# usebeforefree/reed-solomon-cc

Hardware: AMD Instinct MI355X
Metric: device-resident encode+reconstruct GiB/s per GPU (RS(10,4), 1 MiB shards); % HBM roofline (higher is better)
Workload: dtype u8

## Files before the change

include/reedsol.h:

```cpp
#ifndef REEDSOL_AMD_H
#define REEDSOL_AMD_H

#include <stddef.h>
#include <stdint.h>

#ifdef __cplusplus
extern "C" {
#endif

typedef enum rs_status {
  RS_OK = 0,
  RS_ERR_TOO_FEW_ORIGINAL_SHARDS = 1,
  RS_ERR_NOT_ENOUGH_SHARDS = 2,
  RS_ERR_INVALID_SHARD_SIZE = 3,
  RS_ERR_UNSUPPORTED_SHARD_COUNT = 4,
  RS_ERR_TOO_MANY_ORIGINAL_SHARDS = 5,
  RS_ERR_DIFFERENT_SHARD_SIZE = 6,
  RS_ERR_INVALID_SHARD_INDEX = 7,
  RS_ERR_DUPLICATE_SHARD_INDEX = 8,
  RS_ERR_TOO_MANY_SHARDS = 9,
  RS_ERR_OUT_OF_MEMORY = 10,
  RS_ERR_OVERFLOW = 11,
  RS_ERR_LOW_RATE_UNSUPPORTED = 12,
  RS_ERR_SHARD_TAIL_UNSUPPORTED = 13,
// ... 74 lines not shown
                        uint32_t max_u, const uint32_t *d_index, uint64_t index_stride, const void *d_old,
                        const void *d_new, uint64_t change_stripe_stride, void *d_recovery,
                        uint64_t recovery_stripe_stride, int32_t *d_status, uint32_t flags, rs_stream_t stream);
int rs_update_selftest(uint64_t original_count, uint64_t recovery_count, uint32_t max_u, int trials, uint64_t seed,
                       uint64_t *mismatches);

int rs_rebuild_batch_dev(uint64_t original_count, uint64_t recovery_count, size_t shard_bytes, uint64_t n_stripes,
                         const uint8_t *d_present, uint64_t present_stride, uint32_t max_e,
                         const void *d_original, uint64_t original_stripe_stride,
                         const void *d_recovery, uint64_t recovery_stripe_stride,
                         void *d_rebuilt, uint64_t rebuilt_stripe_stride, int32_t *d_status,
                         uint32_t flags, rs_stream_t stream);
const char *rs_rebuild_kernel_name(uint64_t k, uint64_t m, size_t shard_bytes, uint32_t max_e);
int rs_rebuild_compile_check(uint64_t k, uint64_t m, double *compile_ms, uint64_t *code_bytes);
int rs_rebuild_selftest(uint64_t k, uint64_t m, int trials, uint64_t seed, uint64_t *mismatches);

int rs_encode_batch_host(uint64_t original_count, uint64_t recovery_count, size_t shard_bytes, uint64_t n_stripes,
                         const void *h_original, uint64_t original_stripe_stride, void *h_recovery,
                         uint64_t recovery_stripe_stride, uint32_t flags);
int rs_reconstruct_batch_host(uint64_t original_count, uint64_t recovery_count, size_t shard_bytes,
                              uint64_t n_stripes, const uint8_t *present, const void *h_original,
                              uint64_t original_stripe_stride, const void *h_recovery,
                              uint64_t recovery_stripe_stride, void *h_restored, uint64_t restored_stripe_stride,
                              uint32_t flags);

int rs_encode_batch_host_multi(uint64_t original_count, uint64_t recovery_count, size_t shard_bytes,
                               uint64_t n_stripes, const void *h_original, uint64_t original_stripe_stride,
                               void *h_recovery, uint64_t recovery_stripe_stride, uint32_t flags,
                               const int *devices, int n_devices);
int rs_reconstruct_batch_host_multi(uint64_t original_count, uint64_t recovery_count, size_t shard_bytes,
                                    uint64_t n_stripes, const uint8_t *present, const void *h_original,
                                    uint64_t original_stripe_stride, const void *h_recovery,
                                    uint64_t recovery_stripe_stride, void *h_restored,
                                    uint64_t restored_stripe_stride, uint32_t flags, const int *devices,
                                    int n_devices);

const char *rs_encode_kernel_name(uint64_t original_count, uint64_t recovery_count, size_t shard_bytes);
const char *rs_reconstruct_kernel_name(uint64_t original_count, uint64_t recovery_count, size_t shard_bytes,
                                       const uint8_t *present);
const char *rs_patterns_kernel_name(uint64_t original_count, uint64_t recovery_count, size_t shard_bytes,
                                    uint32_t max_e, uint32_t flags);

int rs_net_wait(void);

int rs_reconstruct_warm(uint64_t original_count, uint64_t recovery_count, size_t shard_bytes, const uint8_t *present,
                        uint32_t flags);

const char *rs_last_kernels(void);

int64_t rs_debug_fail_alloc(int64_t n);
int rs_debug_release_caches(uint64_t *pooled_contexts);
int64_t rs_debug_erasure_logs_check(uint64_t k, uint64_t m, const uint8_t *received, int low);
int rs_debug_fft_stamps(uint64_t *out, uint64_t n);

int rs_jit_stats(uint64_t *compiles, uint64_t *cache_hits, uint64_t *modules);

int rs_net_compile_check(uint64_t original_count, uint64_t recovery_count, const uint8_t *present,
                         uint32_t flags, double *compile_ms);

int rs_psyn_compile_check(uint64_t original_count, uint64_t recovery_count, uint32_t flags, double *compile_ms,
                          uint64_t *code_bytes);
int rs_fft_compile_check(uint64_t original_count, uint64_t recovery_count, uint32_t flags, double *compile_ms,
                         uint64_t *code_bytes, uint64_t *valu_ops);
int rs_fft_selftest(uint64_t original_count, uint64_t recovery_count, uint32_t flags, const uint8_t *skip,
                    int trials, uint64_t *mismatches);

int rs_fft_decode_compile_check(uint64_t original_count, uint64_t recovery_count, double *compile_ms,
                                uint64_t *code_bytes);
int rs_fft_pdecode_compile_check(uint64_t original_count, uint64_t recovery_count, const uint8_t *present,
                                 double *compile_ms, uint64_t *code_bytes);
int rs_fft_decode_selftest(uint64_t original_count, uint64_t recovery_count, uint32_t erased, int trials,
                           uint64_t *mismatches);

int rs_lowrate_selftest(uint64_t original_count, uint64_t recovery_count, int trials, uint64_t seed,
                        uint64_t *mismatches);

int rs_engine_fft(uint8_t *shards, uint64_t shard_count, size_t shard_bytes, uint64_t pos, uint64_t size,
                  uint64_t truncated_size, uint64_t skew_delta, uint32_t flags);
int rs_engine_ifft(uint8_t *shards, uint64_t shard_count, size_t shard_bytes, uint64_t pos, uint64_t size,
                   uint64_t truncated_size, uint64_t skew_delta, uint32_t flags);
int rs_engine_mul_scalar(uint8_t *chunks, size_t bytes, uint16_t log_m, uint32_t flags);
int rs_engine_eval_poly(uint16_t *erasures, uint64_t truncated_size);

const uint16_t *rs_table_exp(void);
const uint16_t *rs_table_log(void);
const uint16_t *rs_table_skew(void);
const uint16_t *rs_table_log_walsh(void);
const uint8_t *rs_table_mul_128(void);


#ifdef __cplusplus
}
#endif
#endif
```

reed-solomon-cc_amd/csrc/rs_fftnet.cpp:

```cpp
#include "rs_fftnet.hpp"

#include <algorithm>
#include <cstdio>
#include <cstring>
#include <map>
#include <mutex>
#include <random>
#include <sstream>

#include "reedsol.h"
#include "rs_env.hpp"
#include "rs_gf.hpp"
#include "rs_internal.hpp"

namespace rs {
namespace fftnet {
namespace {

struct Basis {
  bool ok = false;
  uint8_t p[8] = {};
};

const Basis &basis() {
  static const Basis b = [] {
    Basis r;
    const Tables &t = tables();
    r.ok = true;
    for (int i = 0; i < 8; i++) {
      const uint16_t prod = mul16(static_cast<uint16_t>(1u << 8), t.log[1u << i]);
      const uint16_t pi = static_cast<uint16_t>((1u << (8 + i)) ^ prod);
      if (pi >> 8) r.ok = false;
      r.p[i] = static_cast<uint8_t>(pi);
    }
    return r;
  }();
  return b;
}

uint16_t to_uv(uint16_t x) {
  const Basis &b = basis();
  uint8_t lo = 0;
  for (int i = 0; i < 8; i++)
    if (x >> (8 + i) & 1) lo ^= b.p[i];
  return static_cast<uint16_t>(x ^ lo);
}

struct Tw {
  bool zero = true;
  bool sub = false;
  uint8_t A[8] = {}, B[8] = {}, Cm[8] = {}, D[8] = {};
};

Tw twiddle(uint16_t log_m, bool d1) {
  Tw t;
  if (log_m == kModulus) return t;
  t.zero = false;
  for (int j = 0; j < 8; j++) {
    const uint16_t cu = to_uv(mul_engine(to_uv(static_cast<uint16_t>(1u << j)), log_m, d1));
    const uint16_t cv = to_uv(mul_engine(to_uv(static_cast<uint16_t>(1u << (8 + j))), log_m, d1));
    for (int i = 0; i < 8; i++) {
      t.A[i] |= static_cast<uint8_t>((cu >> i & 1) << j);
      t.Cm[i] |= static_cast<uint8_t>((cu >> (8 + i) & 1) << j);
      t.B[i] |= static_cast<uint8_t>((cv >> i & 1) << j);
      t.D[i] |= static_cast<uint8_t>((cv >> (8 + i) & 1) << j);
    }
  }
  t.sub = true;
  for (int i = 0; i < 8; i++)
    if (t.B[i] || t.Cm[i] || t.A[i] != t.D[i]) t.sub = false;
  return t;
}

struct Bf {
  uint32_t x, y;
  uint16_t log_m;
};
struct Layer {
  int bit;
  bool inv;
  std::vector<Bf> bf;
};

uint16_t sk(uint64_t idx) { return idx < kModulus ? tables().skew[idx] : static_cast<uint16_t>(kModulus); }

uint16_t gmul_elem(uint16_t x, uint16_t y) { return x && y ? mul16(x, tables().log[y]) : 0; }

int log2i(uint64_t v) {
  int b = 0;
  while ((1ull << b) < v) b++;
  return b;
}

std::vector<Layer> ifft_layers(uint64_t size, uint64_t trunc, uint64_t sd) {
  std::vector<Layer> out;
  uint64_t d = 1;
  for (uint64_t d4 = 4; d4 <= size; d = d4, d4 <<= 2) {
    Layer l1{log2i(d), true, {}}, l2{log2i(d) + 1, true, {}};
    for (uint64_t r = 0; r < trunc; r += d4) {
      const uint64_t b = r + d + sd - 1;
      const uint16_t m01 = sk(b), m02 = sk(b + d), m23 = sk(b + 2 * d);
      for (uint64_t i = r; i < r + d; i++) {
        l1.bf.push_back({uint32_t(i), uint32_t(i + d), m01});
        l1.bf.push_back({uint32_t(i + 2 * d), uint32_t(i + 3 * d), m23});
        l2.bf.push_back({uint32_t(i), uint32_t(i + 2 * d), m02});
        l2.bf.push_back({uint32_t(i + d), uint32_t(i + 3 * d), m02});
      }
    }
    out.push_back(std::move(l1));
    out.push_back(std::move(l2));
  }
  if (d < size) {
    Layer l{log2i(d), true, {}};
    const uint16_t lm = sk(d + sd - 1);
    for (uint64_t i = 0; i < d; i++) l.bf.push_back({uint32_t(i), uint32_t(d + i), lm});
    out.push_back(std::move(l));
  }
  return out;
}

std::vector<Layer> fft_layers(uint64_t size, uint64_t trunc, uint64_t sd) {
  std::vector<Layer> out;
  uint64_t d4 = size;
  for (uint64_t d = size >> 2; d != 0; d4 = d, d >>= 2) {
// ... 172 lines not shown
#endif
  u32 s[8], o[8];
#pragma unroll
  for (int j = 0; j < 8; j++) s[j] = SWN(x[j]);
#pragma unroll
  for (int i0 = 0; i0 < 8; i0 += RS_RMUL_G) {
    u32 m[16 * RS_RMUL_G];
#pragma unroll
    for (int t = 0; t < 16 * RS_RMUL_G; t++) m[t] = M[16 * i0 + t];
#pragma unroll
    for (int g = 0; g < RS_RMUL_G; g++) {
      u32 a = x[0] & m[16 * g];
#pragma unroll
      for (int j = 1; j < 8; j++) a = __builtin_amdgcn_bitop3_b32(a, x[j], m[16 * g + j], 0x78);
#pragma unroll
      for (int j = 0; j < 8; j++) a = __builtin_amdgcn_bitop3_b32(a, s[j], m[16 * g + 8 + j], 0x78);
      o[i0 + g] = a;
    }
  }
#pragma unroll
  for (int i = 0; i < 8; i++) x[i] = o[i];
}
)HIP";

int sched_of() { return 1; }

int prefetch_of(const Spec &s) {
  return std::max(0, std::min(8, s.prefetch >= 0 ? s.prefetch : env::num(env::FFT_PREFETCH)));
}

int debug_of() { return env::num(env::FFT_DEBUG); }

std::mutex g_stamp_mu;
std::map<int, unsigned long long *> g_stamp_bufs;
unsigned long long *stamp_buffer(int dev) {
  std::lock_guard<std::mutex> lk(g_stamp_mu);
  unsigned long long *&p = g_stamp_bufs[dev];
  if (!p && hipMalloc(reinterpret_cast<void **>(&p), 8 * 64 * 8) == hipSuccess) (void)hipMemset(p, 0, 8 * 64 * 8);
  return p;
}


struct Gen {
  std::ostringstream o;
  int tmp = 0;
  Stats *st = nullptr;
  uint64_t *ops = nullptr;

  std::string fresh(const char *p = "zt") { return p + std::to_string(tmp++); }
  void op(uint64_t n = 1) {
    if (ops) *ops += n;
  }

  void rows(const std::vector<std::string> &ins, const std::vector<uint32_t> &rowmask,
            const std::vector<std::string> &dst, bool acc) {
    std::vector<std::string> names = ins;
    std::vector<std::vector<int>> r(rowmask.size());
    for (size_t i = 0; i < rowmask.size(); i++)
      for (size_t j = 0; j < ins.size(); j++)
        if (rowmask[i] >> j & 1) r[i].push_back(static_cast<int>(j));
    for (;;) {
      std::map<std::pair<int, int>, int> cnt;
      for (auto &row : r)
        for (size_t a = 0; a < row.size(); a++)
          for (size_t b = a + 1; b < row.size(); b++) cnt[{std::min(row[a], row[b]), std::max(row[a], row[b])}]++;
      std::pair<int, int> best{-1, -1};
      int bc = 1;
      for (auto &kv : cnt)
        if (kv.second > bc) {
          bc = kv.second;
          best = kv.first;
        }
      if (best.first < 0) break;
      const std::string nm = fresh();
      o << "  const u32 " << nm << " = " << names[best.first] << " ^ " << names[best.second] << ";\n";
      op();
      const int id = static_cast<int>(names.size());
      names.push_back(nm);
      for (auto &row : r) {
        auto ia = std::find(row.begin(), row.end(), best.first), ib = std::find(row.begin(), row.end(), best.second);
        if (ia != row.end() && ib != row.end()) {
          row.erase(std::remove_if(row.begin(), row.end(), [&](int v) { return v == best.first || v == best.second; }),
                    row.end());
          row.push_back(id);
        }
      }
    }
    for (size_t i = 0; i < r.size(); i++) {
      std::vector<std::string> t;
      for (int id : r[i]) t.push_back(names[id]);
      const std::string &d = dst[i];
      size_t at = 0;
      if (!acc) {
        if (t.empty()) {
          o << "  " << d << " = 0u;\n";
          continue;
        }
        if (t.size() == 1) {
          o << "  " << d << " = " << t[0] << ";\n";
          continue;
        }
        if (t.size() == 2 || t.size() == 4) {
          o << "  " << d << " = " << t[0] << " ^ " << t[1] << ";\n";
          at = 2;
        } else {
          o << "  " << d << " = X3(" << t[0] << ", " << t[1] << ", " << t[2] << ");\n";
          at = 3;
        }
        op();
      }
      for (; at + 1 < t.size(); at += 2) {
        o << "  " << d << " = X3(" << d << ", " << t[at] << ", " << t[at + 1] << ");\n";
        op();
      }
      if (at < t.size()) {
        o << "  " << d << " ^= " << t[at] << ";\n";
        op();
      }
    }
  }

  static std::vector<std::string> regs(const std::string &pfx) {
    std::vector<std::string> v;
    for (int i = 0; i < 8; i++) v.push_back(pfx + "_" + std::to_string(i));
    return v;
  }

  void mul(const std::vector<std::string> &dst, bool acc, const std::vector<std::string> &src, const Tw &t) {
    if (t.sub) {
      if (st) st->subfield++;
      std::vector<uint32_t> rm(8);
      for (int i = 0; i < 8; i++) rm[i] = t.A[i];
      rows(src, rm, dst, acc);
      return;
    }
    if (st) st->general++;
    std::vector<std::string> ins = src;
    for (int j = 0; j < 8; j++) {
      const std::string s = fresh("zs");
      o << "  const u32 " << s << " = SWN(" << src[j] << ");\n";
      op(3);
      ins.push_back(s);
    }
    std::vector<uint32_t> rm(16);
    std::vector<std::string> tl(16);
    for (int i = 0; i < 8; i++) {
      rm[i] = t.A[i] | (uint32_t(t.B[i]) << 8);
      rm[8 + i] = t.D[i] | (uint32_t(t.Cm[i]) << 8);
      tl[i] = fresh("zl");
      tl[8 + i] = fresh("zh");
    }
    o << "  u32 ";
    for (int i = 0; i < 16; i++) o << tl[i] << (i < 15 ? ", " : ";\n");
    rows(ins, rm, tl, false);
    for (int i = 0; i < 8; i++) {
      if (acc)
        o << "  " << dst[i] << " ^= MUX(" << tl[i] << ", " << tl[8 + i] << ", KM.f);\n";
      else
        o << "  " << dst[i] << " = MUX(" << tl[i] << ", " << tl[8 + i] << ", KM.f);\n";
      op(acc ? 2 : 1);
    }
  }

  void pin(const std::vector<std::string> &v) {
    o << "  asm volatile(\"\" :";
    for (size_t i = 0; i < v.size(); i++) o << (i ? ", " : " ") << "\"+v\"(" << v[i] << ")";
    o << ");\n";
  }

  void copy(const std::vector<std::string> &dst, const std::vector<std::string> &src) {
    for (int i = 0; i < 8; i++) o << "  " << dst[i] << " = " << src[i] << ";\n";
  }
  void xor_into(const std::vector<std::string> &dst, const std::vector<std::string> &src) {
    for (int i = 0; i < 8; i++) o << "  " << dst[i] << " ^= " << src[i] << ";\n";
    op(8);
  }

  int sched = 0;
  int nbf = 0;

  void butterfly(const std::string &xn, bool &zx, const std::string &yn, bool &zy, bool inv, const Tw &t) {
    const auto X = regs(xn), Y = regs(yn);
    if (zx && zy) return;
    if (sched && ++nbf % sched == 0) o << "  __builtin_amdgcn_sched_barrier(0);\n";
    if (t.zero && st) st->xor_only++;
    if (inv) {
      if (!zx) {
        if (zy)
          copy(Y, X);
        else
          xor_into(Y, X);
        zy = false;
      }
      if (!t.zero && !zy) {
        mul(X, !zx, Y, t);
        zx = false;
      }
    } else {
      if (!t.zero && !zy) {
        mul(X, !zx, Y, t);
        zx = false;
      }
      if (!zx) {
        if (zy)
          copy(Y, X);
        else
          xor_into(Y, X);
        zy = false;
      }
    }
  }

  void basis_change(const std::vector<std::string> &d) {
    const Basis &b = basis();
    std::vector<std::string> h(8), nn(8);
    for (int i = 0; i < 8; i++) {
      h[i] = fresh("zv");
      o << "  const u32 " << h[i] << " = " << d[i] << " >> 4;\n";
      op();
    }
    std::vector<uint32_t> rm(8, 0);
    for (int j = 0; j < 8; j++)
      for (int i = 0; i < 8; i++)
        if (b.p[i] >> j & 1) rm[j] |= 1u << i;
    o << "  u32 ";
    for (int j = 0; j < 8; j++) {
      nn[j] = fresh("zn");
      o << nn[j] << (j < 7 ? ", " : ";\n");
    }
    rows(h, rm, nn, false);
    for (int j = 0; j < 8; j++)
      if (rm[j]) {
        o << "  " << d[j] << " = XM(" << d[j] << ", " << nn[j] << ");\n";
        op();
      }
  }
};

std::string wname(uint32_t r) { return "w" + std::to_string(r); }
std::string bname(uint32_t t) { return "b" + std::to_string(t); }
std::string cname(uint32_t t) { return "c" + std::to_string(t); }

std::string mask_expr(const std::vector<uint32_t> &per_wave) {
  bool same = true;
  for (uint32_t v : per_wave) same &= v == per_wave[0];
  if (same) return std::to_string(per_wave[0]) + "u";
  std::string e = "0u";
  for (size_t w = per_wave.size(); w-- > 0;)
    e = "(w == " + std::to_string(w) + "u ? " + std::to_string(per_wave[w]) + "u : " + e + ")";
  return e;
}

uint32_t dyn_store_word(const Plan &P) { return static_cast<uint32_t>((P.truncs.size() * P.C + 31) / 32); }

std::string gen_source(const Spec &s, const std::string &name, Stats *stats) {
  Plan P = make_plan(s);
  Gen g;
  g.st = stats;
  g.sched = sched_of();
  Stats dummy;
  if (!g.st) g.st = &dummy;
  std::ostringstream &o = g.o;
  const uint32_t NW = P.NW, C = P.C;
  bool any_xor = s.decode;
  for (uint32_t q = 0; q < s.m; q++) any_xor |= P.out_mode[q] == kOutXorRec;
  const bool dyn = s.dyn;
  const int dbg = debug_of();
  const bool old_order = s.decode && (dbg & 16);
  const bool tail = s.decode && !(dbg & 4);
  const bool spat = s.decode && !s.present.empty();
  std::vector<uint8_t> inR(C, 0);
  std::vector<uint16_t> lp_log(C, 0);
  std::vector<int32_t> out_row(s.k, -1);
  std::vector<uint32_t> cg_log(s.k, 0);
  if (spat) {
    const Tables &T = tables();
    uint32_t e = 0, nr = 0;
// ... 1054 lines not shown
  };
  auto rmul = [](uint16_t x, const uint32_t *M) -> uint16_t {
    const uint8_t u = x & 0xFF, v = x >> 8;
    uint16_t r = 0;
    for (int i = 0; i < 8; i++) {
      int lo = 0, hi = 0;
      for (int j = 0; j < 8; j++) {
        lo ^= ((u >> j & 1) && (M[16 * i + j] & 0x0F0F0F0Fu)) ^ ((v >> j & 1) && (M[16 * i + 8 + j] & 0x0F0F0F0Fu));
        hi ^= ((v >> j & 1) && (M[16 * i + j] & 0xF0F0F0F0u)) ^ ((u >> j & 1) && (M[16 * i + 8 + j] & 0xF0F0F0F0u));
      }
      r |= static_cast<uint16_t>(lo << i | hi << (8 + i));
    }
    return r;
  };
  std::vector<uint32_t> blk(decode_block_words(s));
  for (int tr = 0; tr < trials; tr++) {
    std::vector<uint16_t> data(k), par(m);
    for (auto &x : data) x = static_cast<uint16_t>(rng());
    scalar_encode(data.data(), k, m, false, false, par.data());
    std::vector<uint8_t> present(k + m, 1);
    std::vector<uint32_t> idx(k);
    for (uint32_t i = 0; i < k; i++) idx[i] = i;
    std::shuffle(idx.begin(), idx.end(), rng);
    for (uint32_t i = 0; i < e; i++) present[idx[i]] = 0;
    for (uint32_t p = 0; p < m - e; p++)
      if (rng() % 4 == 0) present[k + rng() % m] = 0;
    uint32_t have = 0;
    for (uint32_t p = 0; p < m; p++) have += present[k + p];
    if (have < e) continue;
    if (decode_block(s, present.data(), blk.data()) != RS_OK) return ~0ull;
    std::vector<uint16_t> d2 = data, enc(m);
    for (uint32_t g = 0; g < k; g++)
      if (!present[g]) d2[g] = 0;
    scalar_encode(d2.data(), k, m, false, false, enc.data());
    std::vector<uint16_t> a(C, 0);
    for (uint32_t p = 0; p < m; p++)
      if (blk[dwm + 1 + p / 32] >> (p % 32) & 1) a[p] = rmul(to_uv(par[p] ^ enc[p]), &blk[mko + 128 * p]);
    for (const Layer &L : ifft_layers(C, m, 0)) apply(a, L);
    for (uint32_t K = 1; K <= (k + C - 1) / C; K++) {
      if (!(blk[dwm] >> K & 1)) continue;
      const uint32_t tK = std::min<uint32_t>(C, k - (K - 1) * C);
      std::vector<uint16_t> y = a;
      for (const Layer &L : fft_layers(C, tK, static_cast<uint64_t>(K) * C)) apply(y, L);
      for (uint32_t q = 0; q < tK; q++) {
        const uint32_t g = (K - 1) * C + q;
        if (present[g]) continue;
        bad += to_uv(rmul(y[q], &blk[mko + 128 * (m + g)])) != data[g];
      }
    }
  }
  return bad;
}

}
}
```

reed-solomon-cc_amd/csrc/rs_fftnet.hpp:

```cpp
#pragma once
#include <hip/hip_runtime.h>

#include <cstdint>
#include <string>
#include <vector>

#include "rs_jit.hpp"

namespace rs {
namespace fftnet {

constexpr uint8_t kOutNone = 0;
constexpr uint8_t kOutStore = 1;
constexpr uint8_t kOutXorRec = 2;

struct Spec {
  uint32_t k = 0, m = 0;
  uint32_t flags = 0;
  std::vector<uint8_t> skip;
  std::vector<uint8_t> out_mode;
  int prefetch = -1;
  uint32_t pieces = 1;
  bool inverse = false;
  bool dyn = false;
  bool decode = false;
  bool blocked = false;
  std::vector<uint8_t> present;
};
uint32_t dyn_mask_words(const Spec &s);

bool supports_inverse(uint64_t k, uint64_t m, uint64_t shard_bytes);

constexpr uint64_t kUnitBytes = 2048;

constexpr uint32_t kMaxChunks = 16;
bool supports(uint64_t k, uint64_t m, uint64_t shard_bytes, bool chunk16 = false);
uint32_t pieces(uint64_t shard_bytes);

std::string generate(const Spec &s, const std::string &name);
std::string cache_key(const Spec &s);
std::string kernel_name(const Spec &s);

const jit::Kernel *get(const Spec &s, bool async, std::string &err, bool &pending);
bool compile_check(const Spec &s, std::string &err, double *ms, size_t *code_bytes);

hipError_t launch(const jit::Kernel &kn, const Spec &s, const uint8_t *data, uint64_t ds, const uint8_t *rec, uint64_t rs,
                  uint8_t *out, uint64_t os, uint64_t sb, uint64_t n_stripes, hipStream_t st,
                  const uint32_t *dmask = nullptr, uint32_t dmask_words = 0, bool shared_mask = false);

uint32_t decode_block_words(const Spec &s);
uint32_t decode_mask_offset(const Spec &s);
bool decode_betas(uint32_t k, uint32_t m, std::vector<uint16_t> &beta);
void scalar_masks(uint16_t c, uint32_t *masks);
void uv_basis(uint32_t p[8]);
int decode_block(const Spec &s, const uint8_t *present, uint32_t *blk);
uint64_t decode_selftest(uint32_t k, uint32_t m, uint32_t e, int trials);

uint64_t selftest(const Spec &s, int trials);
int read_stamps(uint64_t *host, size_t n);

struct Stats {
  uint64_t ops_a = 0, ops_b = 0, ops_io = 0, subfield = 0, general = 0, xor_only = 0;
};
Stats stats(const Spec &s);

}
}
```

reed-solomon-cc_amd/csrc/rs_plans.cpp:

```cpp
#include "rs_host.hpp"

namespace rs {
namespace host {

PlanCache<EncodePlan> g_enc_plans;
PlanCache<DecodePlan> g_dec_plans;

void release_plans() {
  std::lock_guard<std::mutex> lk(g_plan_mu);
  g_enc_plans.clear();
  g_dec_plans.clear();
}

void encode_map(uint64_t k, uint64_t m, uint32_t flags, jit::NetSpec &ns) {
  const bool d1 = flags & RS_FLAG_QUIRK_D1, d2 = flags & RS_FLAG_QUIRK_D2;
  ns.role = "encode";
  ns.n_in = static_cast<uint32_t>(k);
  ns.n_out = static_cast<uint32_t>(m);
  ns.src.clear();
  ns.images.assign(k * m * 16, 0);
  std::vector<uint16_t> in(k, 0), out(m);
  for (uint64_t t = 0; t < k; t++) {
    ns.src.push_back(static_cast<int32_t>(t));
    for (int b = 0; b < 16; b++) {
// ... 487 lines not shown
    return RS_OK;
  });
}

int rs_fft_decode_compile_check(uint64_t k, uint64_t m, double *compile_ms, uint64_t *code_bytes) {
  return guarded([&]() -> int {
    int st = check_codec(k, m, fftnet::kUnitBytes);
    if (st) return st;
    if (!fftnet::supports(k, m, fftnet::kUnitBytes, true)) return fail(RS_ERR_INVALID_ARGUMENT, "no FFT kernel form");
    fftnet::Spec spec;
    spec.k = static_cast<uint32_t>(k);
    spec.m = static_cast<uint32_t>(m);
    spec.dyn = spec.decode = true;
    std::string err;
    size_t bytes = 0;
    if (!fftnet::compile_check(spec, err, compile_ms, &bytes)) return fail(RS_ERR_DEVICE, err);
    if (code_bytes) *code_bytes = bytes;
    return RS_OK;
  });
}

int rs_fft_pdecode_compile_check(uint64_t k, uint64_t m, const uint8_t *present, double *compile_ms,
                                 uint64_t *code_bytes) {
  return guarded([&]() -> int {
    int st = check_codec(k, m, fftnet::kUnitBytes);
    if (st) return st;
    if (!present) return fail(RS_ERR_INVALID_ARGUMENT, "present == NULL");
    if (!fftnet::supports(k, m, fftnet::kUnitBytes, true)) return fail(RS_ERR_INVALID_ARGUMENT, "no FFT kernel form");
    uint64_t e = 0, have = 0;
    for (uint64_t i = 0; i < k; i++) e += present[i] ? 0 : 1;
    for (uint64_t i = 0; i < m; i++) have += present[k + i] ? 1 : 0;
    if (have < e) return fail(RS_ERR_NOT_ENOUGH_SHARDS, "fewer than original_count shards present");
    if (e == 0) return fail(RS_ERR_INVALID_ARGUMENT, "nothing erased");
    fftnet::Spec spec;
    spec.k = static_cast<uint32_t>(k);
    spec.m = static_cast<uint32_t>(m);
    spec.decode = true;
    spec.present.assign(present, present + k + m);
    std::string err;
    size_t bytes = 0;
    if (!fftnet::compile_check(spec, err, compile_ms, &bytes)) return fail(RS_ERR_DEVICE, err);
    if (code_bytes) *code_bytes = bytes;
    return RS_OK;
  });
}

int rs_debug_fft_stamps(uint64_t *out, uint64_t n) {
  return guarded([&]() -> int {
    if (!out) return fail(RS_ERR_INVALID_ARGUMENT, "out == NULL");
    return fftnet::read_stamps(out, n) == 0 ? RS_OK : fail(RS_ERR_DEVICE, "stamp buffer unavailable");
  });
}

int rs_fft_decode_selftest(uint64_t k, uint64_t m, uint32_t e, int trials, uint64_t *mismatches) {
  return guarded([&]() -> int {
    int st = check_codec(k, m, fftnet::kUnitBytes);
    if (st) return st;
    if (!fftnet::supports(k, m, fftnet::kUnitBytes, true) || e > m || e > k || e == 0)
      return fail(RS_ERR_INVALID_ARGUMENT, "no FFT decode form");
    const uint64_t bad = fftnet::decode_selftest(static_cast<uint32_t>(k), static_cast<uint32_t>(m), e, trials);
    if (mismatches) *mismatches = bad;
    return RS_OK;
  });
}

int rs_net_compile_check(uint64_t k, uint64_t m, const uint8_t *present, uint32_t flags, double *compile_ms) {
  return guarded([&]() -> int {
    int st = check_codec(k, m, jit::kUnitBytes);
    if (st) return st;
    jit::NetSpec spec;
    if (present) {
      uint64_t have = 0;
      for (uint64_t i = 0; i < k + m; i++) have += present[i] != 0;
      if (have < k) return fail(RS_ERR_NOT_ENOUGH_SHARDS, "fewer than original_count shards present");
      uint64_t e = 0;
      for (uint64_t i = 0; i < k; i++) e += present[i] ? 0 : 1;
      if (is_low_rate(k, m)) {
        if ((st = low_decode_map(k, m, flags, present, spec))) return st;
      } else if (!jit::supports_async(static_cast<uint32_t>(k), static_cast<uint32_t>(e), jit::kUnitBytes) &&
                 syndrome_pick(k, m, e, flags, jit::kUnitBytes * 64, "auto")) {
        if ((st = syndrome_map(k, m, present, spec))) return st;
      } else {
        reconstruct_map(k, m, flags, present, spec);
      }
    } else if (is_low_rate(k, m)) {
      encode_low_map(k, m, flags, spec);
    } else {
      encode_map(k, m, flags, spec);
    }
    if (!jit::supports_async(spec.n_in, spec.n_out, jit::kUnitBytes))
      return fail(RS_ERR_INVALID_ARGUMENT, "no network form");
    std::string err;
    if (!jit::compile_check(spec, err, compile_ms, nullptr)) return fail(RS_ERR_DEVICE, err);
    return RS_OK;
  });
}

}
```

reed-solomon-cc_amd/reedsol_amd/__init__.py:

```python
from __future__ import annotations

import ctypes as C
import os
from typing import Optional, Sequence

PKG_DIR = os.path.dirname(os.path.dirname(os.path.abspath(__file__)))
LIB_PATH = os.environ.get("RS_AMD_LIB", os.path.join(PKG_DIR, "build", "librs_amd.so"))

FLAG_CORRECTED = 0
FLAG_QUIRK_D1 = 1
FLAG_QUIRK_D2 = 2
FLAG_REF_LITERAL = 3

LOCATE_CLEAN = -1
LOCATE_RECOVERY_SET = -2
LOCATE_UNLOCATED = -3

UPDATE_NONE = 0xFFFFFFFF

_STATUS_NAMES = [
    "Ok", "TooFewOriginalShards", "NotEnoughShards", "InvalidShardSize", "UnsupportedShardCount",
    "TooManyOriginalShards", "DifferentShardSize", "InvalidShardIndex", "DuplicateShardIndex",
    "TooManyShards", "OutOfMemory", "Overflow", "LowRateUnsupported", "ShardTailUnsupported",
    "InvalidArgument", "DeviceError", "NoDevice",
# ... 20 lines not shown
    if not os.path.exists(LIB_PATH):
        raise ImportError(f"librs_amd.so not built: {LIB_PATH} (run __graft_entry__.build())")
    L = C.CDLL(LIB_PATH)
    vp, u8p, u16p, sz, u64, u32 = C.c_void_p, C.POINTER(C.c_uint8), C.POINTER(C.c_uint16), C.c_size_t, \
        C.c_uint64, C.c_uint32
    pp = C.POINTER(C.c_void_p)
    sig = {
        "rs_version": (C.c_char_p, []),
        "rs_status_name": (C.c_char_p, [C.c_int]),
        "rs_last_error": (C.c_char_p, []),
        "rs_use_high_rate": (C.c_int, [u64, u64]),
        "rs_encode": (C.c_int, [u64, u64, sz, pp, pp]),
        "rs_decode": (C.c_int, [u64, u64, sz, pp, pp, pp]),
        "rs_encoder_new": (C.c_int, [u64, u64, sz, C.POINTER(vp)]),
        "rs_encoder_add_original_shard": (C.c_int, [vp, vp, sz]),
        "rs_encoder_encode": (C.c_int, [vp, pp]),
        "rs_encoder_reset": (C.c_int, [vp]),
        "rs_encoder_free": (None, [vp]),
        "rs_decoder_new": (C.c_int, [u64, u64, sz, C.POINTER(vp)]),
        "rs_decoder_add_original_shard": (C.c_int, [vp, u64, vp, sz]),
        "rs_decoder_add_recovery_shard": (C.c_int, [vp, u64, vp, sz]),
        "rs_decoder_decode": (C.c_int, [vp, pp]),
        "rs_decoder_free": (None, [vp]),
        "rs_encode_batch_dev": (C.c_int, [u64, u64, sz, u64, vp, u64, vp, u64, u32, vp]),
        "rs_reconstruct_batch_dev": (C.c_int, [u64, u64, sz, u64, vp, vp, u64, vp, u64, vp, u64, u32, vp]),
        "rs_reconstruct_batch_dev_patterns": (C.c_int, [u64, u64, sz, u64, vp, u64, u32, vp, u64, vp, u64, vp, u64,
                                                        vp, u32, vp]),
        "rs_verify_batch_dev": (C.c_int, [u64, u64, sz, u64, vp, u64, vp, u64, vp, u64, vp, u32, vp]),
        "rs_verify_kernel_name": (C.c_char_p, [u64, u64, sz]),
        "rs_locate_batch_dev": (C.c_int, [u64, u64, sz, u64, vp, u64, vp, u64, vp, vp, u64, vp, u32, vp]),
        "rs_locate_kernel_name": (C.c_char_p, [u64, u64, sz]),
        "rs_locate_selftest": (C.c_int, [u64, u64, C.c_int, u64, vp]),
        "rs_update_batch_dev": (C.c_int, [u64, u64, sz, u64, u32, vp, u64, vp, vp, u64, vp, u64, vp, u32, vp]),
        "rs_update_selftest": (C.c_int, [u64, u64, u32, C.c_int, u64, vp]),
        "rs_rebuild_batch_dev": (C.c_int, [u64, u64, sz, u64, vp, u64, u32, vp, u64, vp, u64, vp, u64, vp, u32, vp]),
        "rs_rebuild_kernel_name": (C.c_char_p, [u64, u64, sz, u32]),
        "rs_rebuild_compile_check": (C.c_int, [u64, u64, vp, vp]),
        "rs_rebuild_selftest": (C.c_int, [u64, u64, C.c_int, u64, vp]),
        "rs_encode_batch_host": (C.c_int, [u64, u64, sz, u64, vp, u64, vp, u64, u32]),
        "rs_reconstruct_batch_host": (C.c_int, [u64, u64, sz, u64, vp, vp, u64, vp, u64, vp, u64, u32]),
        "rs_encode_batch_host_multi": (C.c_int, [u64, u64, sz, u64, vp, u64, vp, u64, u32, vp, C.c_int]),
        "rs_reconstruct_batch_host_multi": (C.c_int, [u64, u64, sz, u64, vp, vp, u64, vp, u64, vp, u64, u32, vp,
                                                      C.c_int]),
        "rs_encode_kernel_name": (C.c_char_p, [u64, u64, sz]),
        "rs_reconstruct_kernel_name": (C.c_char_p, [u64, u64, sz, vp]),
        "rs_net_compile_check": (C.c_int, [u64, u64, vp, u32, vp]),
        "rs_net_wait": (C.c_int, []),
        "rs_reconstruct_warm": (C.c_int, [u64, u64, sz, vp, u32]),
        "rs_last_kernels": (C.c_char_p, []),
        "rs_debug_fail_alloc": (C.c_int64, [C.c_int64]),
        "rs_debug_release_caches": (C.c_int, [vp]),
        "rs_debug_erasure_logs_check": (C.c_int64, [C.c_uint64, C.c_uint64, vp, C.c_int]),
        "rs_debug_fft_stamps": (C.c_int, [vp, u64]),
        "rs_jit_stats": (C.c_int, [vp, vp, vp]),
        "rs_fft_compile_check": (C.c_int, [u64, u64, u32, vp, vp, vp]),
        "rs_psyn_compile_check": (C.c_int, [u64, u64, u32, vp, vp]),
        "rs_patterns_kernel_name": (C.c_char_p, [u64, u64, sz, u32, u32]),
        "rs_fft_selftest": (C.c_int, [u64, u64, u32, vp, C.c_int, vp]),
        "rs_fft_decode_compile_check": (C.c_int, [u64, u64, vp, vp]),
        "rs_fft_pdecode_compile_check": (C.c_int, [u64, u64, vp, vp, vp]),
        "rs_fft_decode_selftest": (C.c_int, [u64, u64, u32, C.c_int, vp]),
        "rs_lowrate_selftest": (C.c_int, [u64, u64, C.c_int, u64, vp]),
        "rs_engine_fft": (C.c_int, [vp, u64, sz, u64, u64, u64, u64, u32]),
        "rs_engine_ifft": (C.c_int, [vp, u64, sz, u64, u64, u64, u64, u32]),
        "rs_engine_mul_scalar": (C.c_int, [vp, sz, C.c_uint16, u32]),
        "rs_engine_eval_poly": (C.c_int, [vp, u64]),
        "rs_table_exp": (u16p, []),
        "rs_table_log": (u16p, []),
        "rs_table_skew": (u16p, []),
        "rs_table_log_walsh": (u16p, []),
        "rs_table_mul_128": (C.POINTER(C.c_uint8), []),
    }
    for name, (res, args) in sig.items():
        f = getattr(L, name)
        f.restype = res
        f.argtypes = args
    _lib = L
    return L


def _check(status: int):
    if status:
        detail = lib().rs_last_error().decode(errors="replace")
        raise _ERRORS.get(status, ReedSolomonError)(detail)


def _buf(b) -> C.Array:
    if isinstance(b, (bytes, bytearray, memoryview)):
        return (C.c_uint8 * len(b)).from_buffer_copy(bytes(b))
    import numpy as np
    a = np.ascontiguousarray(b, dtype=np.uint8)
    return (C.c_uint8 * a.size).from_buffer_copy(a.tobytes())


def use_high_rate(original_count: int, recovery_count: int) -> bool:
    r = lib().rs_use_high_rate(original_count, recovery_count)
    if r < 0:
        _check(-r)
    return bool(r)


def encode(original_count: int, recovery_count: int, original: Sequence[bytes]) -> list:
    if len(original) == 0:
        raise TooFewOriginalShards("no original shards")
    enc = Encoder(original_count, recovery_count, len(original[0]))
    try:
# ... 317 lines not shown
    return ms.value


def jit_stats() -> dict:
    c, h, mo = C.c_uint64(), C.c_uint64(), C.c_uint64()
    _check(lib().rs_jit_stats(C.byref(c), C.byref(h), C.byref(mo)))
    return {"compiles": c.value, "cache_hits": h.value, "modules": mo.value}


def fft_compile_check(k, m, flags=0) -> dict:
    ms, b, ops = C.c_double(), C.c_uint64(), C.c_uint64()
    _check(lib().rs_fft_compile_check(k, m, flags, C.byref(ms), C.byref(b), C.byref(ops)))
    return {"compile_ms": ms.value, "code_bytes": b.value, "valu_ops_per_unit": ops.value}


def psyn_compile_check(k, m, flags=0) -> dict:
    ms, b = C.c_double(), C.c_uint64()
    _check(lib().rs_psyn_compile_check(k, m, flags, C.byref(ms), C.byref(b)))
    return {"compile_ms": ms.value, "code_bytes": b.value}


def lowrate_selftest(k, m, trials=8, seed=1) -> int:
    bad = C.c_uint64()
    _check(lib().rs_lowrate_selftest(k, m, trials, seed, C.byref(bad)))
    return bad.value


def fft_selftest(k, m, flags=0, skip=None, trials=8) -> int:
    bad = C.c_uint64()
    sk = None if skip is None else (C.c_uint8 * k)(*[1 if x else 0 for x in skip])
    _check(lib().rs_fft_selftest(k, m, flags, sk, trials, C.byref(bad)))
    return bad.value


def fft_decode_compile_check(k, m) -> dict:
    ms, b = C.c_double(0), C.c_uint64(0)
    _check(lib().rs_fft_decode_compile_check(k, m, C.byref(ms), C.byref(b)))
    return {"compile_ms": ms.value, "code_bytes": b.value}


def fft_pdecode_compile_check(k, m, present) -> dict:
    ms, b = C.c_double(0), C.c_uint64(0)
    pres = (C.c_uint8 * (k + m))(*[1 if p else 0 for p in present])
    _check(lib().rs_fft_pdecode_compile_check(k, m, pres, C.byref(ms), C.byref(b)))
    return {"compile_ms": ms.value, "code_bytes": b.value}


def fft_decode_selftest(k, m, erased, trials=8) -> int:
    bad = C.c_uint64(0)
    _check(lib().rs_fft_decode_selftest(k, m, erased, trials, C.byref(bad)))
    return bad.value


def net_wait() -> None:
    _check(lib().rs_net_wait())


def reconstruct_warm(k, m, shard_bytes, present, flags: int = FLAG_CORRECTED) -> None:
    pres = (C.c_uint8 * (k + m))(*[1 if p else 0 for p in present])
    _check(lib().rs_reconstruct_warm(k, m, shard_bytes, pres, flags))


def debug_erasure_logs_check(k: int, m: int, received, low: bool = False) -> int:
    buf = (C.c_uint8 * len(received))(*[1 if r else 0 for r in received])
    return int(lib().rs_debug_erasure_logs_check(k, m, buf, 1 if low else 0))


def debug_fail_alloc(n: int) -> int:
    return int(lib().rs_debug_fail_alloc(n))


def debug_release_caches() -> int:
    n = C.c_uint64()
    _check(lib().rs_debug_release_caches(C.byref(n)))
    return n.value


def debug_fft_stamps():
    import numpy as np
    a = np.zeros(8 * 64, np.uint64)
    _check(lib().rs_debug_fft_stamps(a.ctypes.data_as(C.c_void_p), a.size))
    return a.reshape(8, 64)


def last_kernels() -> list:
    t = lib().rs_last_kernels().decode()
    return t.split(";") if t else []


def engine_fft(shards: bytearray, shard_count, shard_bytes, pos, size, trunc, skew_delta, flags=0, inverse=False):
    buf = (C.c_uint8 * len(shards)).from_buffer(shards)
    f = lib().rs_engine_ifft if inverse else lib().rs_engine_fft
    _check(f(C.addressof(buf), shard_count, shard_bytes, pos, size, trunc, skew_delta, flags))


def engine_mul_scalar(chunks: bytearray, log_m: int, flags=0):
    buf = (C.c_uint8 * len(chunks)).from_buffer(chunks)
    _check(lib().rs_engine_mul_scalar(C.addressof(buf), len(chunks), log_m, flags))


def engine_eval_poly(erasures, truncated_size: int):
    _check(lib().rs_engine_eval_poly(erasures.ctypes.data_as(C.c_void_p), truncated_size))


def table(name: str):
    import numpy as np
# ... 9 lines not shown
```

Before: 4046.

## Replace greedy XOR-pair CSE with search-based XOR network synthesis for GF multiplies

Replaces the pairwise-greedy common-subexpression pass that emits XOR networks for the bitsliced GF(2^16) twiddle multiplies with a memoised synthesiser. It tries pair, triple and random-walk greedy searches with a cost model that counts 3-input XORs, and folds the accumulate input into the network where that saves an op. The goal is fewer VALU XOR instructions per butterfly in the JIT-generated FFT kernels. The cost is extra host-side synthesis time at JIT compile, plus a new self-check entry point that verifies the networks.

```diff
diff --git a/include/reedsol.h b/include/reedsol.h
--- a/include/reedsol.h
+++ b/include/reedsol.h
@@ -150,6 +150,8 @@
 int rs_debug_release_caches(uint64_t *pooled_contexts);
 int64_t rs_debug_erasure_logs_check(uint64_t k, uint64_t m, const uint8_t *received, int low);
 int rs_debug_fft_stamps(uint64_t *out, uint64_t n);
+int rs_debug_netsynth_check(uint64_t original_count, uint64_t recovery_count, uint32_t flags, int trials,
+                            uint64_t *matrices, uint64_t *ops, uint64_t *mismatches);
 
 int rs_jit_stats(uint64_t *compiles, uint64_t *cache_hits, uint64_t *modules);
 
diff --git a/reed-solomon-cc_amd/csrc/rs_fftnet.cpp b/reed-solomon-cc_amd/csrc/rs_fftnet.cpp
--- a/reed-solomon-cc_amd/csrc/rs_fftnet.cpp
+++ b/reed-solomon-cc_amd/csrc/rs_fftnet.cpp
@@ -70,6 +70,254 @@
   for (int i = 0; i < 8; i++)
     if (t.B[i] || t.Cm[i] || t.A[i] != t.D[i]) t.sub = false;
   return t;
+}
+
+constexpr int kNetOut = 1000, kNetExt = 2000;
+struct NetOp {
+  int dst, a, b, c;
+};
+struct NetProg {
+  int nin = 0, nout = 0, ntmp = 0, cost = 0;
+  std::vector<uint8_t> ext;
+  std::vector<NetOp> ops;
+};
+enum NetForm { kNetSet = 0, kNetAcc = 1, kNetBlocks = 2, kNetBlocksAcc = 3 };
+
+struct Synth {
+  int nin = 0;
+  NetForm form = kNetSet;
+  int cap = 0;
+  std::vector<uint64_t> row;
+  std::vector<uint64_t> gate;
+  static int pc(uint64_t v) { return __builtin_popcountll(v); }
+  int nsig() const { return nin + static_cast<int>(gate.size()); }
+  int terms(size_t i) const { return pc(row[i]) + (form == kNetAcc ? 1 : 0); }
+
+  std::vector<uint8_t> ext() const {
+    std::vector<uint8_t> e(row.size(), form == kNetAcc ? 1 : 0);
+    if (form == kNetBlocksAcc)
+      for (size_t i = 0; i < 8; i++)
+        if (pc(row[i]) % 2 == 0 && pc(row[8 + i]) % 2 == 0) e[i] = e[8 + i] = 1;
+    return e;
+  }
+  int cost() const {
+    int c = 0;
+    for (uint64_t g : gate) c += pc(g) >> 1;
+    const std::vector<uint8_t> e = ext();
+    for (size_t i = 0; i < row.size(); i++) c += (pc(row[i]) + e[i]) >> 1;
+    if (form == kNetBlocks) c += 8;
+    if (form == kNetBlocksAcc)
+      for (size_t i = 0; i < 8; i++) c += e[i] ? 1 : 2;
+    return c;
+  }
+  int delta(uint64_t g, int *rows_in = nullptr) const {
+    const int s = pc(g);
+    int d = s >> 1, n = 0;
+    for (size_t i = 0; i < row.size(); i++)
+      if ((row[i] & g) == g) {
+        const int t = terms(i);
+        d += ((t - s + 1) >> 1) - (t >> 1);
+        n++;
+      }
+    if (rows_in) *rows_in = n;
+    return d;
+  }
+  void take(uint64_t g) {
+    const uint64_t bit = 1ull << nsig();
+    for (uint64_t &r : row)
+      if ((r & g) == g) r = (r & ~g) | bit;
+    gate.push_back(g);
+  }
+  bool room() const { return static_cast<int>(gate.size()) < cap && nsig() < 63; }
+
+  template <class F>
+  void candidates(bool triples, F &&f) const {
+    const int n = nsig();
+    uint8_t cnt[64][64] = {};
+    for (uint64_t r : row)
+      for (int a = 0; a < n; a++)
+        if (r >> a & 1)
+          for (int b = a + 1; b < n; b++)
+            if (r >> b & 1) cnt[a][b]++;
+    for (int a = 0; a < n; a++)
+      for (int b = a + 1; b < n; b++) {
+        if (cnt[a][b] < 2) continue;
+        f((1ull << a) | (1ull << b));
+        if (!triples) continue;
+        for (int c = b + 1; c < n; c++)
+          if (cnt[a][c] >= 2 && cnt[b][c] >= 2) f((1ull << a) | (1ull << b) | (1ull << c));
+      }
+    if (!triples) return;
+    for (size_t i = 0; i < row.size(); i++)
+      for (size_t j = i + 1; j < row.size(); j++)
+        if (pc(row[i] & row[j]) >= 4) f(row[i] & row[j]);
+  }
+
+  void pair_greedy() {
+    while (room()) {
+      uint64_t best = 0;
+      int bc = 1;
+      candidates(false, [&](uint64_t g) {
+        int n = 0;
+        for (uint64_t r : row) n += (r & g) == g;
+        if (n > bc) bc = n, best = g;
+      });
+      if (!best) break;
+      take(best);
+    }
+  }
+  void greedy(bool triples) {
+    while (room()) {
+      uint64_t best = 0;
+      int bd = 0, bn = 0;
+      candidates(triples, [&](uint64_t g) {
+        int n = 0;
+        const int d = delta(g, &n);
+        if (d < bd || (d == bd && d < 0 && n > bn)) bd = d, bn = n, best = g;
+      });
+      if (!best) break;
+      take(best);
+    }
+  }
+  void random_walk(std::mt19937 &rng) {
+    std::vector<uint64_t> bestg, okg;
+    int flat = 0;
+    while (room()) {
+      bestg.clear();
+      okg.clear();
+      int bd = 0;
+      candidates(true, [&](uint64_t g) {
+        const int d = delta(g);
+        if (d > 0) return;
+        okg.push_back(g);
+        if (d < bd) bd = d, bestg.clear();
+        if (d == bd) bestg.push_back(g);
+      });
+      if (okg.empty()) break;
+      const bool any = rng() % 4 == 0;
+      const std::vector<uint64_t> &from = any ? okg : bestg;
+      const uint64_t g = from[rng() % from.size()];
+      if (delta(g) == 0 && ++flat > 4) break;
+      take(g);
+    }
+  }
+  void tidy() {
+    for (bool again = true; again;) {
+      again = false;
+      for (int t = static_cast<int>(gate.size()) - 1; t >= 0; t--) {
+        const uint64_t bit = 1ull << (nin + t), lo = bit - 1;
+        int users = 0;
+        uint64_t *u = nullptr;
+        for (uint64_t &r : row)
+          if (r & bit) users++, u = &r;
+        for (uint64_t &g : gate)
+          if (g & bit) users++, u = &g;
+        if (users > 1) continue;
+        if (users == 1) *u ^= bit ^ gate[t];
+        auto squeeze = [&](uint64_t m) { return (m & lo) | ((m >> 1) & ~lo); };
+        gate.erase(gate.begin() + t);
+        for (uint64_t &r : row) r = squeeze(r);
+        for (uint64_t &g : gate) g = squeeze(g);
+        again = true;
+      }
+    }
+  }
+
+  NetProg program() const {
+    NetProg p;
+    p.nin = nin;
+    p.nout = static_cast<int>(row.size());
+    p.ntmp = static_cast<int>(gate.size());
+    p.ext = ext();
+    p.cost = cost();
+    std::vector<uint8_t> born(gate.size(), 0);
+    auto chain = [&](int dst, std::vector<int> t) {
+      if (t.empty()) return p.ops.push_back({dst, -1, -1, -1});
+      if (t.size() == 1) return p.ops.push_back({dst, t[0], -1, -1});
+      size_t at = t.size() >= 3 ? 3 : 2;
+      p.ops.push_back({dst, t[0], t[1], at == 3 ? t[2] : -1});
+      for (; at < t.size(); at += 2) p.ops.push_back({dst, dst, t[at], at + 1 < t.size() ? t[at + 1] : -1});
+    };
+    auto sigs = [&](uint64_t m) {
+      std::vector<int> t;
+      for (int s = 0; s < nsig(); s++)
+        if (m >> s & 1) t.push_back(s);
+      return t;
+    };
+    auto need = [&](auto &&self, uint64_t m) -> void {
+      for (int s : sigs(m)) {
+        if (s < nin || born[s - nin]) continue;
+        self(self, gate[s - nin]);
+        born[s - nin] = 1;
+        chain(s, sigs(gate[s - nin]));
+      }
+    };
+    for (size_t i = 0; i < row.size(); i++) {
+      need(need, row[i]);
+      std::vector<int> t;
+      if (p.ext[i]) t.push_back(kNetExt + static_cast<int>(i));
+      for (int s : sigs(row[i])) t.push_back(s);
+      const bool same = form == kNetAcc;
+      if (same && t.size() == 1) continue;
+      chain(kNetOut + static_cast<int>(i), t);
+    }
+    return p;
+  }
+};
+
+const NetProg &synthesise(const std::vector<uint32_t> &rowmask, int nin, NetForm form, int cap) {
+  static std::mutex mu;
+  static std::map<std::pair<std::vector<uint32_t>, std::vector<int>>, NetProg> memo;
+  std::lock_guard<std::mutex> lk(mu);
+  const std::pair<std::vector<uint32_t>, std::vector<int>> key{rowmask, {nin, form, cap}};
+  auto it = memo.find(key);
+  if (it != memo.end()) return it->second;
+  Synth base;
+  base.nin = nin;
+  base.form = form;
+  base.cap = cap;
+  for (uint32_t r : rowmask) base.row.push_back(r);
+  Synth best = base;
+  best.pair_greedy();
+  auto offer = [&](Synth &s) {
+    s.tidy();
+    if (s.cost() < best.cost() || (s.cost() == best.cost() && s.gate.size() < best.gate.size())) best = s;
+  };
+  for (int triples = 0; triples < 2; triples++) {
+    Synth s = base;
+    s.greedy(triples != 0);
+    offer(s);
+  }
+  uint32_t seed = 0x9E3779B9u;
+  for (uint32_t r : rowmask) seed = (seed ^ r) * 0x01000193u;
+  std::mt19937 rng(seed);
+  const int restarts = rowmask.size() > 8 ? 8 : 96;
+  for (int i = 0; i < restarts; i++) {
+    Synth s = base;
+    s.random_walk(rng);
+    offer(s);
+  }
+  return memo.emplace(key, best.program()).first->second;
+}
+
+constexpr int kNetCap8 = 10, kNetCap16 = 20;
+
+std::vector<uint32_t> basis_rows() {
+  std::vector<uint32_t> rm(8, 0);
+  for (int j = 0; j < 8; j++)
+    for (int i = 0; i < 8; i++)
+      if (basis().p[i] >> j & 1) rm[j] |= 1u << i;
+  return rm;
+}
+
+const NetProg &mul_prog(const Tw &t, bool acc) {
+  std::vector<uint32_t> rm(t.sub ? 8 : 16);
+  for (int i = 0; i < 8; i++) {
+    rm[i] = t.sub ? t.A[i] : t.A[i] | (uint32_t(t.B[i]) << 8);
+    if (!t.sub) rm[8 + i] = t.D[i] | (uint32_t(t.Cm[i]) << 8);
+  }
+  if (t.sub) return synthesise(rm, 8, acc ? kNetAcc : kNetSet, kNetCap8);
+  return synthesise(rm, 16, acc ? kNetBlocksAcc : kNetBlocks, kNetCap16);
 }
 
 struct Bf {
@@ -348,72 +596,27 @@
     if (ops) *ops += n;
   }
 
+  void emit(const NetProg &p, const std::vector<std::string> &ins, const std::vector<std::string> &dst,
+            const std::vector<std::string> &ext) {
+    std::vector<std::string> tn(p.ntmp);
+    auto nm = [&](int id) -> const std::string & {
+      return id >= kNetExt ? ext[id - kNetExt] : id >= kNetOut ? dst[id - kNetOut] : id >= p.nin ? tn[id - p.nin] : ins[id];
+    };
+    for (const NetOp &q : p.ops) {
+      o << "  ";
+      if (q.dst < kNetOut && tn[q.dst - p.nin].empty()) o << "u32 " << (tn[q.dst - p.nin] = fresh());
+      else o << nm(q.dst);
+      if (q.a < 0) o << " = 0u;\n";
+      else if (q.b < 0) o << " = " << nm(q.a) << ";\n";
+      else if (q.c < 0) o << " = " << nm(q.a) << " ^ " << nm(q.b) << ";\n";
+      else o << " = X3(" << nm(q.a) << ", " << nm(q.b) << ", " << nm(q.c) << ");\n";
+      if (q.b >= 0) op();
+    }
+  }
+
   void rows(const std::vector<std::string> &ins, const std::vector<uint32_t> &rowmask,
             const std::vector<std::string> &dst, bool acc) {
-    std::vector<std::string> names = ins;
-    std::vector<std::vector<int>> r(rowmask.size());
-    for (size_t i = 0; i < rowmask.size(); i++)
-      for (size_t j = 0; j < ins.size(); j++)
-        if (rowmask[i] >> j & 1) r[i].push_back(static_cast<int>(j));
-    for (;;) {
-      std::map<std::pair<int, int>, int> cnt;
-      for (auto &row : r)
-        for (size_t a = 0; a < row.size(); a++)
-          for (size_t b = a + 1; b < row.size(); b++) cnt[{std::min(row[a], row[b]), std::max(row[a], row[b])}]++;
-      std::pair<int, int> best{-1, -1};
-      int bc = 1;
-      for (auto &kv : cnt)
-        if (kv.second > bc) {
-          bc = kv.second;
-          best = kv.first;
-        }
-      if (best.first < 0) break;
-      const std::string nm = fresh();
-      o << "  const u32 " << nm << " = " << names[best.first] << " ^ " << names[best.second] << ";\n";
-      op();
-      const int id = static_cast<int>(names.size());
-      names.push_back(nm);
-      for (auto &row : r) {
-        auto ia = std::find(row.begin(), row.end(), best.first), ib = std::find(row.begin(), row.end(), best.second);
-        if (ia != row.end() && ib != row.end()) {
-          row.erase(std::remove_if(row.begin(), row.end(), [&](int v) { return v == best.first || v == best.second; }),
-                    row.end());
-          row.push_back(id);
-        }
-      }
-    }
-    for (size_t i = 0; i < r.size(); i++) {
-      std::vector<std::string> t;
-      for (int id : r[i]) t.push_back(names[id]);
-      const std::string &d = dst[i];
-      size_t at = 0;
-      if (!acc) {
-        if (t.empty()) {
-          o << "  " << d << " = 0u;\n";
-          continue;
-        }
-        if (t.size() == 1) {
-          o << "  " << d << " = " << t[0] << ";\n";
-          continue;
-        }
-        if (t.size() == 2 || t.size() == 4) {
-          o << "  " << d << " = " << t[0] << " ^ " << t[1] << ";\n";
-          at = 2;
-        } else {
-          o << "  " << d << " = X3(" << t[0] << ", " << t[1] << ", " << t[2] << ");\n";
-          at = 3;
-        }
-        op();
-      }
-      for (; at + 1 < t.size(); at += 2) {
-        o << "  " << d << " = X3(" << d << ", " << t[at] << ", " << t[at + 1] << ");\n";
-        op();
-      }
-      if (at < t.size()) {
-        o << "  " << d << " ^= " << t[at] << ";\n";
-        op();
-      }
-    }
+    emit(synthesise(rowmask, static_cast<int>(ins.size()), acc ? kNetAcc : kNetSet, kNetCap8), ins, dst, dst);
   }
 
   static std::vector<std::string> regs(const std::string &pfx) {
@@ -423,11 +626,10 @@
   }
 
   void mul(const std::vector<std::string> &dst, bool acc, const std::vector<std::string> &src, const Tw &t) {
+    const NetProg &p = mul_prog(t, acc);
     if (t.sub) {
       if (st) st->subfield++;
-      std::vector<uint32_t> rm(8);
-      for (int i = 0; i < 8; i++) rm[i] = t.A[i];
-      rows(src, rm, dst, acc);
+      emit(p, src, dst, dst);
       return;
     }
     if (st) st->general++;
@@ -438,23 +640,19 @@
       op(3);
       ins.push_back(s);
     }
-    std::vector<uint32_t> rm(16);
-    std::vector<std::string> tl(16);
+    std::vector<std::string> tl(16), ext(16);
     for (int i = 0; i < 8; i++) {
-      rm[i] = t.A[i] | (uint32_t(t.B[i]) << 8);
-      rm[8 + i] = t.D[i] | (uint32_t(t.Cm[i]) << 8);
       tl[i] = fresh("zl");
       tl[8 + i] = fresh("zh");
+      ext[i] = ext[8 + i] = dst[i];
     }
     o << "  u32 ";
     for (int i = 0; i < 16; i++) o << tl[i] << (i < 15 ? ", " : ";\n");
-    rows(ins, rm, tl, false);
+    emit(p, ins, tl, ext);
     for (int i = 0; i < 8; i++) {
-      if (acc)
-        o << "  " << dst[i] << " ^= MUX(" << tl[i] << ", " << tl[8 + i] << ", KM.f);\n";
-      else
-        o << "  " << dst[i] << " = MUX(" << tl[i] << ", " << tl[8 + i] << ", KM.f);\n";
-      op(acc ? 2 : 1);
+      const bool x = acc && !p.ext[i];
+      o << "  " << dst[i] << (x ? " ^= MUX(" : " = MUX(") << tl[i] << ", " << tl[8 + i] << ", KM.f);\n";
+      op(x ? 2 : 1);
     }
   }
 
@@ -508,17 +706,13 @@
   }
 
   void basis_change(const std::vector<std::string> &d) {
-    const Basis &b = basis();
     std::vector<std::string> h(8), nn(8);
     for (int i = 0; i < 8; i++) {
       h[i] = fresh("zv");
       o << "  const u32 " << h[i] << " = " << d[i] << " >> 4;\n";
       op();
     }
-    std::vector<uint32_t> rm(8, 0);
-    for (int j = 0; j < 8; j++)
-      for (int i = 0; i < 8; i++)
-        if (b.p[i] >> j & 1) rm[j] |= 1u << i;
+    const std::vector<uint32_t> rm = basis_rows();
     o << "  u32 ";
     for (int j = 0; j < 8; j++) {
       nn[j] = fresh("zn");
@@ -1679,5 +1873,114 @@
   return bad;
 }
 
-}
-}
+namespace {
+void run_prog(const NetProg &p, const uint32_t *in, const uint32_t *ext, uint32_t *out) {
+  std::vector<uint32_t> tmp(p.ntmp, 0);
+  auto val = [&](int id) -> uint32_t {
+    return id < 0 ? 0u : id >= kNetExt ? ext[id - kNetExt] : id >= kNetOut ? out[id - kNetOut] : id >= p.nin ? tmp[id - p.nin] : in[id];
+  };
+  for (const NetOp &q : p.ops) {
+    const uint32_t v = val(q.a) ^ val(q.b) ^ val(q.c);
+    (q.dst >= kNetOut ? out[q.dst - kNetOut] : tmp[q.dst - p.nin]) = v;
+  }
+}
+
+uint64_t check_mul(const Tw &t, int trials, std::mt19937_64 &rng) {
+  constexpr uint32_t F = 0x0F0F0F0Fu;
+  uint64_t bad = 0;
+  for (int acc = 0; acc < 2; acc++) {
+    const NetProg &p = mul_prog(t, acc != 0);
+    for (int tr = 0; tr < trials; tr++) {
+      uint32_t y[16], x[16], want[8], got[8];
+      for (int i = 0; i < 8; i++) {
+        y[i] = static_cast<uint32_t>(rng());
+        y[8 + i] = (y[i] >> 4 & F) | (y[i] << 4 & ~F);
+        x[i] = x[8 + i] = static_cast<uint32_t>(rng());
+      }
+      for (int i = 0; i < 8; i++) {
+        uint32_t lo = 0, hi = 0;
+        for (int j = 0; j < 8; j++) {
+          const uint32_t u = y[j] & F, v = y[j] >> 4 & F;
+          lo ^= (t.A[i] >> j & 1 ? u : 0u) ^ (t.B[i] >> j & 1 ? v : 0u);
+          hi ^= (t.Cm[i] >> j & 1 ? u : 0u) ^ (t.D[i] >> j & 1 ? v : 0u);
+        }
+        want[i] = (lo | hi << 4) ^ (acc ? x[i] : 0u);
+      }
+      if (t.sub) {
+        for (int i = 0; i < 8; i++) got[i] = acc ? x[i] : ~want[i];
+        run_prog(p, y, x, got);
+      } else {
+        uint32_t tl[16];
+        for (int i = 0; i < 16; i++) tl[i] = ~0u;
+        run_prog(p, y, x, tl);
+        for (int i = 0; i < 8; i++) got[i] = ((tl[i] & F) | (tl[8 + i] & ~F)) ^ (acc && !p.ext[i] ? x[i] : 0u);
+      }
+      for (int i = 0; i < 8; i++) bad += got[i] != want[i];
+    }
+  }
+  return bad;
+}
+}
+
+uint64_t netsynth_check(uint32_t k, uint32_t m, uint32_t flags, int trials, uint64_t *matrices, uint64_t *ops) {
+  std::mt19937_64 rng(4242 + k * 131 + m);
+  const bool d1 = (flags & RS_FLAG_QUIRK_D1) != 0;
+  std::vector<uint16_t> logs;
+  if (k == 0) {
+    for (uint32_t i = 0; i < 255; i++) logs.push_back(static_cast<uint16_t>(257 * i));
+    for (int i = 0; i < 64; i++) logs.push_back(static_cast<uint16_t>(rng() % kModulus));
+  } else {
+    const uint32_t C = static_cast<uint32_t>(ceil_pow2(m));
+    std::vector<std::vector<Layer>> all;
+    Spec s;
+    s.k = k;
+    s.m = m;
+    s.flags = flags;
+    for (int inv = 0; inv < 2; inv++) {
+      if (inv && !supports_inverse(k, m, kUnitBytes)) break;
+      s.inverse = inv != 0;
+      const Plan P = make_plan(s);
+      all.insert(all.end(), P.ifft.begin(), P.ifft.end());
+      all.push_back(P.fft);
+    }
+    all.push_back(ifft_layers(C, m, 0));
+    for (uint32_t K = 1; K <= (k + C - 1) / C; K++)
+      all.push_back(fft_layers(C, std::min<uint32_t>(C, k - (K - 1) * C), static_cast<uint64_t>(K) * C));
+    for (const auto &ls : all)
+      for (const Layer &L : ls)
+        for (const Bf &b : L.bf)
+          if (b.log_m != kModulus) logs.push_back(b.log_m);
+    std::sort(logs.begin(), logs.end());
+    logs.erase(std::unique(logs.begin(), logs.end()), logs.end());
+  }
+  uint64_t bad = 0, n = 0, cost = 0;
+  for (uint16_t l : logs) {
+    const Tw t = twiddle(l, d1);
+    if (k == 0 && !d1 && n < 2 * 255 && !t.sub) return ~0ull;
+    bad += check_mul(t, trials, rng);
+    cost += mul_prog(t, false).cost + mul_prog(t, true).cost;
+    n += 2;
+  }
+  if (k == 0) {
+    const std::vector<uint32_t> rm = basis_rows();
+    const NetProg &p = synthesise(rm, 8, kNetSet, kNetCap8);
+    for (int tr = 0; tr < trials; tr++) {
+      uint32_t h[8], got[8];
+      for (int i = 0; i < 8; i++) h[i] = static_cast<uint32_t>(rng()), got[i] = ~0u;
+      run_prog(p, h, h, got);
+      for (int j = 0; j < 8; j++) {
+        uint32_t want = 0;
+        for (int i = 0; i < 8; i++) want ^= rm[j] >> i & 1 ? h[i] : 0u;
+        bad += got[j] != want;
+      }
+    }
+    cost += p.cost;
+    n++;
+  }
+  if (matrices) *matrices = n;
+  if (ops) *ops = cost;
+  return bad;
+}
+
+}
+}
diff --git a/reed-solomon-cc_amd/csrc/rs_fftnet.hpp b/reed-solomon-cc_amd/csrc/rs_fftnet.hpp
--- a/reed-solomon-cc_amd/csrc/rs_fftnet.hpp
+++ b/reed-solomon-cc_amd/csrc/rs_fftnet.hpp
@@ -57,6 +57,7 @@
 uint64_t decode_selftest(uint32_t k, uint32_t m, uint32_t e, int trials);
 
 uint64_t selftest(const Spec &s, int trials);
+uint64_t netsynth_check(uint32_t k, uint32_t m, uint32_t flags, int trials, uint64_t *matrices, uint64_t *ops);
 int read_stamps(uint64_t *host, size_t n);
 
 struct Stats {
diff --git a/reed-solomon-cc_amd/csrc/rs_plans.cpp b/reed-solomon-cc_amd/csrc/rs_plans.cpp
--- a/reed-solomon-cc_amd/csrc/rs_plans.cpp
+++ b/reed-solomon-cc_amd/csrc/rs_plans.cpp
@@ -563,6 +563,21 @@
   });
 }
 
+int rs_debug_netsynth_check(uint64_t k, uint64_t m, uint32_t flags, int trials, uint64_t *matrices, uint64_t *ops,
+                            uint64_t *mismatches) {
+  return guarded([&]() -> int {
+    if (k || m) {
+      int st = check_codec(k, m, fftnet::kUnitBytes);
+      if (st) return st;
+      if (!fftnet::supports(k, m, fftnet::kUnitBytes, true)) return fail(RS_ERR_INVALID_ARGUMENT, "no FFT kernel form");
+    }
+    const uint64_t bad =
+        fftnet::netsynth_check(static_cast<uint32_t>(k), static_cast<uint32_t>(m), flags, trials, matrices, ops);
+    if (mismatches) *mismatches = bad;
+    return RS_OK;
+  });
+}
+
 int rs_fft_decode_selftest(uint64_t k, uint64_t m, uint32_t e, int trials, uint64_t *mismatches) {
   return guarded([&]() -> int {
     int st = check_codec(k, m, fftnet::kUnitBytes);
diff --git a/reed-solomon-cc_amd/reedsol_amd/__init__.py b/reed-solomon-cc_amd/reedsol_amd/__init__.py
--- a/reed-solomon-cc_amd/reedsol_amd/__init__.py
+++ b/reed-solomon-cc_amd/reedsol_amd/__init__.py
@@ -96,6 +96,7 @@
         "rs_debug_release_caches": (C.c_int, [vp]),
         "rs_debug_erasure_logs_check": (C.c_int64, [C.c_uint64, C.c_uint64, vp, C.c_int]),
         "rs_debug_fft_stamps": (C.c_int, [vp, u64]),
+        "rs_debug_netsynth_check": (C.c_int, [u64, u64, u32, C.c_int, vp, vp, vp]),
         "rs_jit_stats": (C.c_int, [vp, vp, vp]),
         "rs_fft_compile_check": (C.c_int, [u64, u64, u32, vp, vp, vp]),
         "rs_psyn_compile_check": (C.c_int, [u64, u64, u32, vp, vp]),
@@ -519,6 +520,12 @@
     return bad.value
 
 
+def debug_netsynth_check(k=0, m=0, flags=0, trials=4) -> dict:
+    n, ops, bad = C.c_uint64(0), C.c_uint64(0), C.c_uint64(0)
+    _check(lib().rs_debug_netsynth_check(k, m, flags, trials, C.byref(n), C.byref(ops), C.byref(bad)))
+    return {"matrices": n.value, "ops": ops.value, "mismatches": bad.value}
+
+
 def net_wait() -> None:
     _check(lib().rs_net_wait())
 
```

After: 4045, median of 4. About the same (-0.0%).
